# Balajimcr/MuLUT

Measured on AMD Instinct MI355X. Metric: Mpixels/sec SR-x4 2-stage sdy LUT inference (HR output pixels; LR-in = value/16), higher is better.
Workload: dtype u8; 1 GPU; 2-stage sdy x4, 128 x LR 1080x1920x3 -> HR 4320x7680x3 per GPU per step in 4 launches of 32 frames, D-natural; batch=32 draws, repeated in order to 128 frames, frames_per_gpu=128, frames_per_launch=32, stages=2, modes=sdy, scale=4, luts=shipped sr_x2sdy fine-tuned int8 tables, parallelism=frames sharded over 1 GPU(s), no collective

## Files before the change

mulut_amd/csrc/mulut_core.h:

```cpp
#ifndef MULUT_CORE_H_
#define MULUT_CORE_H_

#include <stdint.h>

#if defined(__HIPCC__)
#define MULUT_HD __host__ __device__ __forceinline__
#else
#define MULUT_HD static inline
#endif

namespace mulut {

template <int IV>
struct IvGeom {
    static_assert(IV >= 4 && IV <= 6, "sampling intervals 4, 5 and 6");
    static constexpr int q = 1 << IV;
    static constexpr int L = (1 << (8 - IV)) + 1;
    static constexpr int sA = L * L * L, sB = L * L, sC = L, sD = 1;
    static constexpr int rows = L * L * L * L;
    static constexpr int all = sA + sB + sC + sD;
};
MULUT_HD constexpr int interval_rows(int interval) {
    return interval == 4 ? IvGeom<4>::rows : interval == 5 ? IvGeom<5>::rows : interval == 6 ? IvGeom<6>::rows : 0;
}
// ... 532 lines not shown
    const uint32_t c0 = k0 & 0x0FFF0FFFu;
    const uint32_t c1 = c0 + (k1 & 0x0FFF0FFFu);
    const uint32_t c2 = c1 + (k2 & 0x0FFF0FFFu);
    o.cum[0] = pk_mad(pk_shr11(c0), pk_dup((uint32_t)kStrideA - kFullMark), c0);
    o.cum[1] = pk_mad(pk_shr11(c1), pk_dup((uint32_t)kStrideA - kFullMark), c1);
    o.cum[2] = pk_mad(pk_shr11(c2), pk_dup((uint32_t)kStrideA - kFullMark), c2);
    o.w[0] = pk_dup(kQ) - f1;
    o.w[1] = f1 - f2;
    o.w[2] = f2 - f3;
    o.w[3] = f3 - f4;
    o.w[4] = f4;
}
MULUT_HD void full_pair1_rows(const FullPair1 &p, int half, uint32_t (&r)[5]) {
    const uint32_t b = half ? (p.base >> 16) : (p.base & 0xFFFFu);
    r[0] = b;
    for (int j = 0; j < 3; ++j) {
        r[j + 1] = b + (half ? (p.cum[j] >> 16) : (p.cum[j] & 0xFFFFu));
    }
    r[4] = b + (uint32_t)kAllStrides;
}

MULUT_HD uint32_t bytes_3_1(uint32_t x) {
#if defined(__HIP_DEVICE_COMPILE__)
    return __builtin_amdgcn_perm(0u, x, 0x0C010C03u);
#else
    return (x >> 24) | (((x >> 8) & 0xFFu) << 16);
#endif
}
MULUT_HD uint32_t bytes_2_0(uint32_t x) {
#if defined(__HIP_DEVICE_COMPILE__)
    return __builtin_amdgcn_perm(0u, x, 0x0C000C02u);
#else
    return ((x >> 16) & 0xFFu) | ((x & 0xFFu) << 16);
#endif
}
MULUT_HD void swar_fma_rev4(uint32_t (&lo)[4], uint32_t (&hi)[4], const uint32_t (&row)[4], uint32_t w) {
    for (int k = 0; k < 4; ++k) {
        lo[3 - k] += bytes_3_1(row[k]) * w;
        hi[3 - k] += bytes_2_0(row[k]) * w;
    }
}

template <int HALF>
MULUT_HD void swar_fma_rev4_pk(uint32_t (&lo)[4], uint32_t (&hi)[4], const uint32_t (&row)[4], uint32_t wpk) {
    for (int k = 0; k < 4; ++k) {
        lo[3 - k] = pk_mad_w<HALF>(bytes_3_1(row[k]), wpk, lo[3 - k]);
        hi[3 - k] = pk_mad_w<HALF>(bytes_2_0(row[k]), wpk, hi[3 - k]);
    }
}

template <int HALF>
MULUT_HD uint32_t pk_mad_w_swap(uint32_t x, uint32_t wpk, uint32_t acc) {
#if defined(__HIP_DEVICE_COMPILE__)
    const mulut_u16x2 wv = MULUT_PK(wpk);
    const mulut_u16x2 ws = __builtin_shufflevector(wv, wv, HALF, HALF);
    const mulut_u16x2 xv = MULUT_PK(x);
    return MULUT_UNPK(__builtin_shufflevector(xv, xv, 1, 0) * ws + MULUT_PK(acc));
#else
    return pk_mad_w<HALF>((x >> 16) | (x << 16), wpk, acc);
#endif
}
template <int HALF>
MULUT_HD void swar_fma_x4(uint32_t (&lo)[4], uint32_t (&hi)[4], const uint32_t (&rlo)[4], const uint32_t (&rhi)[4], uint32_t wpk) {
    for (int k = 0; k < 4; ++k) {
        lo[k] = pk_mad_w<HALF>(rlo[k], wpk, lo[k]);
        hi[k] = pk_mad_w<HALF>(rhi[k], wpk, hi[k]);
    }
}
template <int HALF>
MULUT_HD void swar_fma_x4_rev(uint32_t (&lo)[4], uint32_t (&hi)[4], const uint32_t (&rlo)[4], const uint32_t (&rhi)[4], uint32_t wpk) {
    for (int k = 0; k < 4; ++k) {
        lo[3 - k] = pk_mad_w_swap<HALF>(rhi[k], wpk, lo[3 - k]);
        hi[3 - k] = pk_mad_w_swap<HALF>(rlo[k], wpk, hi[3 - k]);
    }
}

MULUT_HD void combine_pairs4(const uint32_t (&lo02)[4], const uint32_t (&hi02)[4], const uint32_t (&lo13)[4],
                             const uint32_t (&hi13)[4], uint32_t (&lo)[4], uint32_t (&hi)[4]) {
    lo[0] = lo02[0] + ((lo13[3] & 0xFFFFu) | (lo13[1] << 16));
    hi[0] = hi02[0] + ((lo13[2] & 0xFFFFu) | (lo13[0] << 16));
    lo[1] = lo02[1] + ((hi13[3] & 0xFFFFu) | (hi13[1] << 16));
    hi[1] = hi02[1] + ((hi13[2] & 0xFFFFu) | (hi13[0] << 16));
    lo[2] = lo02[2] + ((lo13[3] >> 16) | (lo13[1] & 0xFFFF0000u));
    hi[2] = hi02[2] + ((lo13[2] >> 16) | (lo13[0] & 0xFFFF0000u));
    lo[3] = lo02[3] + ((hi13[3] >> 16) | (hi13[1] & 0xFFFF0000u));
    hi[3] = hi02[3] + ((hi13[2] >> 16) | (hi13[0] & 0xFFFF0000u));
}

MULUT_HD uint32_t rhe_clip_u8_f32(int K, float inv_d) {
#if defined(__HIP_DEVICE_COMPILE__)
    const float q = __builtin_rintf((float)K * inv_d);
    return __builtin_amdgcn_cvt_pk_u8_f32(q, 0u, 0u);
#else
    const float q = __builtin_rintf((float)K * inv_d);
    return q < 0.0f ? 0u : (q > 255.0f ? 255u : (uint32_t)q);
#endif
}

MULUT_HD uint32_t rhe_pack4_f32(int K0, int K1, int K2, int K3, float inv_d) {
#if defined(__HIP_DEVICE_COMPILE__)
    uint32_t r = __builtin_amdgcn_cvt_pk_u8_f32(__builtin_rintf((float)K0 * inv_d), 0u, 0u);
    r = __builtin_amdgcn_cvt_pk_u8_f32(__builtin_rintf((float)K1 * inv_d), 1u, r);
    r = __builtin_amdgcn_cvt_pk_u8_f32(__builtin_rintf((float)K2 * inv_d), 2u, r);
    r = __builtin_amdgcn_cvt_pk_u8_f32(__builtin_rintf((float)K3 * inv_d), 3u, r);
    return r;
#else
    return rhe_clip_u8_f32(K0, inv_d) | (rhe_clip_u8_f32(K1, inv_d) << 8) | (rhe_clip_u8_f32(K2, inv_d) << 16) |
           (rhe_clip_u8_f32(K3, inv_d) << 24);
#endif
}

MULUT_HD uint32_t rhe_clip_u8_fma(uint32_t S, float inv_d, float c) {
    const float q = __builtin_rintf(__builtin_fmaf((float)S, inv_d, c));
#if defined(__HIP_DEVICE_COMPILE__)
    return __builtin_amdgcn_cvt_pk_u8_f32(q, 0u, 0u);
#else
    return q < 0.0f ? 0u : (q > 255.0f ? 255u : (uint32_t)q);
#endif
}
MULUT_HD uint32_t rhe_pack4_fma(uint32_t S0, uint32_t S1, uint32_t S2, uint32_t S3, float inv_d, float c) {
#if defined(__HIP_DEVICE_COMPILE__)
    uint32_t r = __builtin_amdgcn_cvt_pk_u8_f32(__builtin_fmaf((float)S0, inv_d, c), 0u, 0u);
    r = __builtin_amdgcn_cvt_pk_u8_f32(__builtin_fmaf((float)S1, inv_d, c), 1u, r);
    r = __builtin_amdgcn_cvt_pk_u8_f32(__builtin_fmaf((float)S2, inv_d, c), 2u, r);
    r = __builtin_amdgcn_cvt_pk_u8_f32(__builtin_fmaf((float)S3, inv_d, c), 3u, r);
    return r;
#else
    return rhe_clip_u8_fma(S0, inv_d, c) | (rhe_clip_u8_fma(S1, inv_d, c) << 8) | (rhe_clip_u8_fma(S2, inv_d, c) << 16) |
           (rhe_clip_u8_fma(S3, inv_d, c) << 24);
#endif
}
MULUT_HD bool rhe_fma_valid(uint32_t smax, int unbias, DivMagic m, float inv_d, float c) {
    for (uint32_t s = 0; s <= smax; ++s)
        if (rhe_clip_u8_fma(s, inv_d, c) != rhe_clip_u8((int)s - unbias, m)) return false;
    return true;
}

MULUT_HD uint32_t rhe_clip_u8_fma_i(int K, float inv_d, float c) {
    const float q = __builtin_rintf(__builtin_fmaf((float)K, inv_d, c));
    return q < 0.0f ? 0u : (q > 255.0f ? 255u : (uint32_t)q);
}
MULUT_HD bool rhe_fma_valid_i(int kmin, int kmax, int bias, DivMagic m, float inv_d, float c) {
    for (int k = kmin; k <= kmax; ++k)
        if (rhe_clip_u8_fma_i(k, inv_d, c) != rhe_clip_u8(k + bias, m)) return false;
    return true;
}

MULUT_HD bool rhe_f32_valid(int kmin, int kmax, DivMagic m, float inv_d) {
    for (int k = kmin; k <= kmax; ++k)
        if (rhe_clip_u8_f32(k, inv_d) != rhe_clip_u8(k, m)) return false;
    return true;
}

}
#endif
```

mulut_amd/csrc/mulut_kernels.hip:

```cpp
#include <hip/hip_runtime.h>
#include <string.h>

#include <mutex>
#include <set>
#include <utility>

#include "mulut_dev.h"
#include "mulut_interval.h"

namespace mulut {

template <int IV>
__device__ __forceinline__ int pass_value(const void *lut, int idx, int u, int e) {
    if (IV == kInterval && u > 1) return (int)((const uint8_t *)lut)[(long long)idx * (row_dwords(u) * 4) + e] - 128;
    return (int)((const int8_t *)lut)[(long long)idx * iv_row_bytes(u) + e];
}

template <int IV>
__global__ void __launch_bounds__(256) pass_kernel(PassArgs a) {
    const long long nsite = (long long)a.C * a.H * a.W;
    const long long s = (long long)blockIdx.x * blockDim.x + threadIdx.x;
    if (s >= nsite) return;
    const int x = (int)(s % a.W);
    const int y = (int)((s / a.W) % a.H);
// ... 394 lines not shown
    const uint32_t pd = w[(2 + yd) * PW + 2 + xd] | ((uint32_t)w[(2 - yd) * PW + 2 - xd] << 16);
    TubePair bp;
    simplex4_tube_pair<false>(k0, ha16, base_a, pb, pc, pd, bp);
    dirty |= bp.t_oob;
    tube_rows<R, 0, IMM>(smem, bp, acc);
    tube_rows<R + 2, 1, IMM>(smem, bp, acc);
}

template <int PAT, int PW>
__device__ __forceinline__ void tube_mode(const uint8_t *smem, uint32_t win, uint32_t k0, uint32_t ha16, uint32_t ha27, RotAcc<4> &acc, uint32_t &dirty) {
    const uint32_t base_a = ha27 + pk_dup((uint32_t)tube_bias(PAT));
    tube_pair<PAT, 0, PW>(smem, win, k0, ha16, base_a, acc, dirty);
    tube_pair<PAT, 1, PW>(smem, win, k0, ha16, base_a, acc, dirty);
}

template <int OUT, int TW, int TH>
__global__ void __launch_bounds__(TW *TH) stage_tube_kernel(StageArgs a, BandArgs b) {
    constexpr int PW = TW + 2 * kTubeHaloX, PH = TH + 2 * kHalo;
    constexpr int NT = TW * TH;
    constexpr int DW = PW / 4, PER4 = (3 * PH * DW + NT - 1) / NT;
    static_assert(((2 * 3 * PH * PW + 15) / 16) * 16 == kTubeTileBytes, "tile buffer size");
    extern __shared__ __attribute__((aligned(16))) uint8_t smem[];

    const int tx = threadIdx.x % TW, ty = threadIdx.x / TW;
    const int ntiles = a.N * a.tiles_x * a.tiles_y;
    const int G = gridDim.x;
    const bool by_xcd = (G & 7) == 0;
    const int per = (ntiles + 7) >> 3;
    const int first = by_xcd ? (int)(blockIdx.x & 7) * per + (int)(blockIdx.x >> 3) : (int)blockIdx.x;
    const int last = by_xcd ? imin(((int)(blockIdx.x & 7) + 1) * per, ntiles) : ntiles;
    const int step = by_xcd ? (G >> 3) : G;
    auto next_tile = [&](int t) {
        if (a.verdict_take >= 0)
            while (t < last && (int)a.verdict[t] != a.verdict_take) t += step;
        return t;
    };
    const int total = a.C * PH * PW;
    const int ylo = imax(a.oy0 - kHalo, 0), yhi = imin(a.oy1 + kHalo, a.H) - 1;
    const bool dw_ok = a.in.sX == 1 && ((a.W | a.in.sY | a.in.sC) & 3) == 0 && (a.in.sN & 3) == 0 && (((uintptr_t)a.in.p) & 3) == 0;
    auto fetch = [&](int tile, uint32_t (&v)[PER4]) {
        if (!dw_ok) return;
        int n, y0, x0;
        decode_tile(a, tile, n, y0, x0, TW, TH);
#pragma unroll
        for (int k = 0; k < PER4; ++k) {
            const int i = (int)threadIdx.x + k * NT;
            const int q = i % DW, py = (i / DW) % PH, c = imin(i / (DW * PH), a.C - 1);
            const int gy = imin(imax(y0 + py - kHalo, ylo), yhi);
            const int gx = imin(imax(x0 - kTubeHaloX + 4 * q, 0), a.W - 4);
            v[k] = *(const uint32_t *)view_addr(a.in, n, c, gy, gx);
        }
    };
    auto stash = [&](int tile, int buf, const uint32_t (&v)[PER4]) {
        int n, y0, x0;
        decode_tile(a, tile, n, y0, x0, TW, TH);
        uint8_t *dst = smem + 3 * kTubeBandBytes + buf * kTubeTileBytes;
        if (dw_ok) {
            int tid = (int)threadIdx.x;
            asm volatile("" : "+v"(tid));
#pragma unroll
            for (int k = 0; k < PER4; ++k) {
                const int i = tid + k * NT;
                if (i < a.C * PH * DW) {
                    const int gx = x0 - kTubeHaloX + 4 * (i % DW);
                    const uint32_t sel_lo = gx < 0 ? 0x0C000C00u : gx > a.W - 4 ? 0x0C030C03u : 0x0C010C00u;
                    const uint32_t sel_hi = gx < 0 ? 0x0C000C00u : gx > a.W - 4 ? 0x0C030C03u : 0x0C030C02u;
                    const uint32_t lo = __builtin_amdgcn_perm(0u, v[k], sel_lo), hi = __builtin_amdgcn_perm(0u, v[k], sel_hi);
                    uint2 c2;
                    c2.x = pk_mad(lo, pk_dup(0x1001u), 0u) & 0xF0F0F0F0u;
                    c2.y = pk_mad(hi, pk_dup(0x1001u), 0u) & 0xF0F0F0F0u;
                    *(uint2 *)(dst + 8 * i) = c2;
                }
            }
        } else {
            for (int i = threadIdx.x; i < total; i += NT) {
                const int px = i % PW, py = (i / PW) % PH, c = i / (PW * PH);
                const int gy = imin(imax(y0 + py - kHalo, ylo), yhi);
                const int gx = imin(imax(x0 + px - kTubeHaloX, 0), a.W - 1);
                ((uint16_t *)dst)[i] = (uint16_t)pixel_code(*view_addr(a.in, n, c, gy, gx));
            }
        }
    };

    int tile = next_tile(first);
    if (tile >= last) return;
    uint32_t pix[PER4];
    fetch(tile, pix);
    for (int m = 0; m < a.M; ++m) {
        const int pat = a.dj[m][0] == 2 ? 1 : a.di[m][0] == 1 ? 2 : 0;
        const uint4 *src = (const uint4 *)b.band[m];
        uint4 *dst = (uint4 *)(smem + pat * kTubeBandBytes);
        for (int i = threadIdx.x; i < kTubeBandBytes / 16; i += NT) dst[i] = src[i];
    }
    stash(tile, 0, pix);
    __syncthreads();

    for (int it = 0; tile < last; ++it) {
        const int nxt = next_tile(tile + step);
        if (nxt < last) fetch(nxt, pix);
        int n, y0, x0;
        decode_tile(a, tile, n, y0, x0, TW, TH);
        const int y = y0 + ty, x = x0 + tx;
        if (y < a.oy1 && x < a.W) {
            uint32_t win = (uint32_t)(3 * kTubeBandBytes + (it & 1) * kTubeTileBytes + 2 * (ty * PW + tx + kTubeHaloX - kHalo));
            uint32_t o0[4], o1[4], o2[4];
#pragma unroll
            for (int k = 0; k < 4; ++k) o0[k] = o1[k] = o2[k] = 0;
            uint32_t dmask = 0u;
#pragma clang loop unroll(disable)
            for (int c = 0; c < a.C; ++c, win += 2 * PH * PW) {
                uint32_t dirty = 0u;
                const uint32_t ca = *(const uint16_t *)(smem + win + 2 * (2 * PW + 2));
                const uint32_t k0 = tube_anchor_key(ca), ha16 = tube_anchor_h16(ca), ha27 = pk_mad(ha16, pk_dup(kTubeSA), 0u);
                RotAcc<4> acc;
                acc.clear();
                for (int mv = 0; mv < a.M; ++mv) {
                    const int m = __builtin_amdgcn_readfirstlane(mv);
                    const int pat = a.dj[m][0] == 2 ? 1 : a.di[m][0] == 1 ? 2 : 0;
                    if (pat == 0) tube_mode<0, PW>(smem, win, k0, ha16, ha27, acc, dirty);
                    else if (pat == 1) tube_mode<1, PW>(smem, win, k0, ha16, ha27, acc, dirty);
                    else tube_mode<2, PW>(smem, win, k0, ha16, ha27, acc, dirty);
                }
                if constexpr (OUT == kOutPackedRGBU4) {
#pragma unroll
                    for (int k = 0; k < 4; ++k) { o0[k] = o1[k]; o1[k] = o2[k]; }
                    tube_finish_rows(a, acc, o2);
                } else {
                    uint32_t o[4];
                    finish_channel<4, OUT>(a, acc, n, c, y, x, o);
                }
                dmask |= (dirty != 0u ? 1u : 0u) << c;
            }
            if constexpr (OUT == kOutPackedRGBU4) store_rgb<4>(a, n, y, x, o0, o1, o2);
            if (__ballot(dmask != 0u) != 0ull) {
                const uint32_t pixel_id = ((uint32_t)n * (uint32_t)a.H + (uint32_t)y) * (uint32_t)a.W + (uint32_t)x;
                for (int c = 0; c < a.C; ++c) {
                    const bool d = ((dmask >> c) & 1u) != 0u;
                    const unsigned long long dm = __ballot(d);
                    if (dm == 0ull) continue;
                    const int lane = (int)(threadIdx.x & 63);
                    uint32_t at = 0;
                    if (lane == __ffsll((long long)dm) - 1) at = atomicAdd(a.fix_count, (uint32_t)__popcll(dm));
                    at = (uint32_t)__shfl((int)at, __ffsll((long long)dm) - 1);
                    if (d) a.fix_list[at + (uint32_t)__popcll(dm & ((1ull << lane) - 1ull))] = pixel_id | ((uint32_t)c << 30);
                }
            }
        }
        if (nxt < last) stash(nxt, (it + 1) & 1, pix);
        __syncthreads();
        tile = nxt;
    }
}

__global__ void __launch_bounds__(256) stage_up_fix2_kernel(StageArgs a) {
    __shared__ int s_sum[16][16];
    const uint32_t count = *a.fix_count;
    const int grp = (int)(threadIdx.x >> 4), ln = (int)(threadIdx.x & 15);
    const int ylo = imax(a.oy0 - kHalo, 0), yhi = imin(a.oy1 + kHalo, a.H) - 1;
    const int unbias = 128 * kQ * 4 * a.M - a.bias_num;
    for (uint32_t i = blockIdx.x * 16u + (uint32_t)grp; i < count; i += gridDim.x * 16u) {
        const uint32_t ent = a.fix_list[i], id = ent & 0x3FFFFFFFu, only = ent >> 30;
        const int x = (int)(id % (uint32_t)a.W), y = (int)((id / (uint32_t)a.W) % (uint32_t)a.H), n = (int)(id / ((uint32_t)a.W * (uint32_t)a.H));
        if (n >= a.N || y < a.oy0 || y >= a.oy1) continue;
        const int c_lo = only == 3u ? 0 : (int)only, c_hi = only == 3u ? imin(a.C, 3) : imin((int)only + 1, a.C);
        for (int c = c_lo; c < c_hi; ++c) {
            s_sum[grp][ln] = 0;
            __builtin_amdgcn_fence(__ATOMIC_RELEASE, "wavefront");
            auto px = [&](int dy, int dx) {
                const int gy = imin(imax(y + dy, ylo), yhi), gx = imin(imax(x + dx, 0), a.W - 1);
                return (int)*view_addr(a.in, n, c, gy, gx);
            };
            const int va = px(0, 0);
            for (int p = ln; p < 4 * a.M; p += 16) {
                const int m = p >> 2, r = p & 3;
                int dy, dx, v[3];
#pragma unroll
                for (int k = 0; k < 3; ++k) {
                    sample_offset(r, a.di[m][k], a.dj[m][k], dy, dx);
                    v[k] = px(dy, dx);
                }
                int idx[5], w[5];
                simplex4(va, v[0], v[1], v[2], idx, w);
                const uint4 *tab = (const uint4 *)a.lut[m];
                uint32_t row[5][4];
#pragma unroll
                for (int j = 0; j < 5; ++j) {
                    const uint4 t = tab[idx[j]];
                    row[j][0] = t.x; row[j][1] = t.y; row[j][2] = t.z; row[j][3] = t.w;
                }
#pragma unroll
                for (int e = 0; e < 16; ++e) {
                    int sum = 0;
#pragma unroll
                    for (int j = 0; j < 5; ++j) sum += w[j] * (int)((row[j][e >> 2] >> (8 * (e & 3))) & 0xFFu);
                    const int pos = r == 0 ? e : r == 1 ? (e & 3) * 4 + 3 - (e >> 2) : r == 2 ? 15 - e : (3 - (e & 3)) * 4 + (e >> 2);
                    atomicAdd(&s_sum[grp][pos], sum);
                }
            }
            __builtin_amdgcn_fence(__ATOMIC_ACQ_REL, "wavefront");
            const uint32_t b = rhe_clip_u8(s_sum[grp][ln] - unbias, a.div);
            *const_cast<uint8_t *>(view_addr(a.out, n, c, y * 4 + (ln >> 2), x * 4 + (ln & 3))) = (uint8_t)b;
            __builtin_amdgcn_fence(__ATOMIC_ACQ_REL, "wavefront");
        }
    }
}

hipError_t launch_stage_up_fix(const StageArgs &a, int num_cus, hipStream_t st) {
    if (a.C > 3 || !a.fix_list || !a.fix_count) return hipErrorInvalidValue;
    hipLaunchKernelGGL(stage_up_fix2_kernel, dim3((unsigned)(8 * num_cus)), dim3(256), 0, st, a);
    return hipGetLastError();
}

const char *stage_tube_name(int out_mode) {
    return out_mode == kOutPackedRGBU4 ? "stage_tube_kernel<rgb>" : out_mode == kOutPlanarU4 ? "stage_tube_kernel<planar>"
                                                                                              : "stage_tube_kernel<generic>";
}

template <int OUT>
static hipError_t launch_tube_t(const StageArgs &a, const BandArgs &b, int num_cus, hipStream_t st) {
    auto kern = stage_tube_kernel<OUT, KB_TW, KB_TH>;
    {
        const hipError_t e = raise_lds_limit((const void *)kern, 160 * 1024);
        if (e != hipSuccess) return e;
    }
    const long long ntiles = (long long)a.N * a.tiles_x * a.tiles_y;
    if (ntiles <= 0 || ntiles > 0x7fffffffLL) return hipErrorInvalidValue;
    const unsigned grid = (unsigned)(ntiles < num_cus ? ntiles : num_cus);
    hipLaunchKernelGGL(kern, dim3(grid), dim3(KB_TW * KB_TH), (size_t)kTubeLdsBytes, st, a, b);
    return hipGetLastError();
}

hipError_t launch_stage_tube(const StageArgs &a, const BandArgs &b, int out_mode, int num_cus, hipStream_t st) {
    if (a.C > 3 || a.M > 3) return hipErrorInvalidValue;
    if (out_mode == kOutPlanarU4) return launch_tube_t<kOutPlanarU4>(a, b, num_cus, st);
    if (out_mode == kOutPackedRGBU4 && a.C == 3) return launch_tube_t<kOutPackedRGBU4>(a, b, num_cus, st);
    return launch_tube_t<kOutGeneric>(a, b, num_cus, st);
}

#if defined(MULUT_TUBE2_ASM_INC)
#include MULUT_TUBE2_ASM_INC
#else
#include "mulut_tube2_asm.inc"
#endif

struct T2Pair {
    uint32_t base, s0, s1, s2;
    uint32_t w0, w1, w2, w3, w4;
};
__host__ __device__ constexpr int t2_modes(int pats) { return pats & 3; }
__host__ __device__ constexpr int t2_pat(int pats, int m) { return (pats >> (2 + 2 * m)) & 3; }
constexpr int kT2W = 16, kT2H = 4;
constexpr int kT2PW = kT2W + 2 * kTubeHaloX, kT2PH = kT2H + 2 * kHalo, kT2Chan = 2 * kT2PH * kT2PW;
constexpr int kT2WaveTileBytes = 3 * kT2Chan;
constexpr int kT2FixCap = 3 * kT2W * kT2H;
constexpr int kT2FixOff = 3 * kTubeBandBytes + 16 * kT2WaveTileBytes + 2 * 16 * KB_TW * KB_TH;
constexpr int kTube2LdsBytes = kT2FixOff + 16 * kT2FixCap * 4 + 16;
static_assert(kTube2LdsBytes <= 160 * 1024, "LDS budget");
static_assert(KB_TW % kT2W == 0 && KB_TH % kT2H == 0 && (KB_TW / kT2W) * (KB_TH / kT2H) == 16 && KB_TW / kT2W == 4, "16 wave tiles per verdict tile, four across");
__host__ __device__ constexpr int t2_nb(int pat, int r, int k, int sign) {
    return 2 * ((2 + sign * rot_dy(r, kPatDi[pat][k], kPatDj[pat][k])) * kT2PW + 2 + sign * rot_dx(r, kPatDi[pat][k], kPatDj[pat][k]));
}
__host__ __device__ constexpr int t2_imm(int pat) { return pat * kTubeBandBytes - tube_bias(pat); }

__device__ __forceinline__ float t2_f32_of_i16(uint32_t x) {
    float f;
    asm("v_cvt_f32_i32_sdwa %0, sext(%1) dst_sel:DWORD dst_unused:UNUSED_PAD src0_sel:WORD_0" : "=v"(f) : "v"(x));
    return f;
}

template <int PAT>
__device__ __forceinline__ void t2_index(uint32_t k0, uint32_t ha, uint32_t base_a0, uint32_t pb, uint32_t pc, uint32_t pd, T2Pair &o, uint32_t &dirty, bool test) {
    constexpr uint32_t SB = kTubeSB * 16, SC = kTubeSC * 16, SD = kTubeSD * 16;
    uint32_t k1 = pb | pk_dup(SB), k2 = pc | pk_dup(SC), k3 = pd | pk_dup(SD);
    pk_cmpx_desc(k0, k1);
    pk_cmpx_desc(k2, k3);
    pk_cmpx_desc(k0, k2);
    pk_cmpx_desc(k1, k3);
    pk_cmpx_desc(k1, k2);
    const uint32_t f1 = pk_shr12(k0), f2 = pk_shr12(k1), f3 = pk_shr12(k2), f4 = pk_shr12(k3);
    o.base = pk_mad(pb, pk_dup(SB), pk_mad(pc, pk_dup(SC), pk_mad(pd, pk_dup(SD), base_a0 + pk_dup((uint32_t)tube_bias(PAT)))));
    o.s0 = k0 & 0x0FF00FF0u;
    o.s1 = k1 & 0x0FF00FF0u;
    o.s2 = k2 & 0x0FF00FF0u;
    o.w0 = pk_dup(kQ) - f1;
    o.w1 = f1 - f2;
    o.w2 = f2 - f3;
    o.w3 = f3 - f4;
    o.w4 = f4;
    if (test) {
        asm volatile("; MULUT_T2_TUBE_TEST");
        const uint32_t hb = pb & 0x000F000Fu, hc = pc & 0x000F000Fu, hd = pd & 0x000F000Fu;
        const uint32_t mx = pk_max(pk_max(hb, hc), pk_max(hd, ha));
        const uint32_t mn = pk_min(pk_min(hb, hc), pk_min(hd, ha));
        dirty |= (mx - mn) & 0xFFFEFFFEu;
    }
}

#define T2_ACC_OPS(lo, hi) [l0] "+v"(lo[0]), [l1] "+v"(lo[1]), [l2] "+v"(lo[2]), [l3] "+v"(lo[3]), [h0] "+v"(hi[0]), [h1] "+v"(hi[1]), [h2] "+v"(hi[2]), [h3] "+v"(hi[3])
#define T2_TMP_OPS [a0] "=&v"(a0), [a1] "=&v"(a1), [a2] "=&v"(a2), [a3] "=&v"(a3)
#define T2_W_OPS(c) [w0] "v"(c.w0), [w1] "v"(c.w1), [w2] "v"(c.w2), [w3] "v"(c.w3), [w4] "v"(c.w4)
#define T2_ADDR_OPS(n) [base] "v"(n.base), [s0] "v"(n.s0), [s1] "v"(n.s1), [s2] "v"(n.s2)
#define T2_IMM_OPS(PAT) [ilo] "i"(t2_imm(PAT)), [ihi] "i"(t2_imm(PAT) + kTubePlaneBytes), [ilo4] "i"(t2_imm(PAT) + kTubeAll * 16), [ihi4] "i"(t2_imm(PAT) + kTubeAll * 16 + kTubePlaneBytes)
#define T2_NB_OPS(PAT, R, OFF) [n0] "i"(t2_nb(PAT, R, 0, 1) + (OFF)), [n1] "i"(t2_nb(PAT, R, 0, -1) + (OFF)), [n2] "i"(t2_nb(PAT, R, 1, 1) + (OFF)), \
    [n3] "i"(t2_nb(PAT, R, 1, -1) + (OFF)), [n4] "i"(t2_nb(PAT, R, 2, 1) + (OFF)), [n5] "i"(t2_nb(PAT, R, 2, -1) + (OFF)), [nan] "i"(2 * (2 * kT2PW + 2) + (OFF))

#define T2_NBOUT_OPS [pb] "=&v"(pb), [pc] "=&v"(pc), [pd] "=&v"(pd), [t0] "=&v"(t0), [t1] "=&v"(t1), [t2] "=&v"(t2)
template <int PAT, int FORM>
__device__ __forceinline__ void t2_block_a(uint32_t (&lo)[4], uint32_t (&hi)[4], const T2Pair &cur) {
    uint32_t a0, a1, a2, a3;
#define T2_A_STMT(BLK) asm volatile(BLK : T2_ACC_OPS(lo, hi), T2_TMP_OPS : T2_W_OPS(cur), T2_ADDR_OPS(cur), T2_IMM_OPS(PAT) : TUBE2_CLOBBERS)
    if constexpr (FORM < 0) T2_A_STMT(TUBE2_ASM_A);
    else if constexpr (FORM == 0) T2_A_STMT(TUBE2_ASM1_A_R0);
    else T2_A_STMT(TUBE2_ASM1_A_R1);
#undef T2_A_STMT
}
template <int FORM, int NPAT, int NN, int TPAT, int TR, int TOFF, bool LAST>
__device__ __forceinline__ void t2_block_b(uint32_t (&lo)[4], uint32_t (&hi)[4], const T2Pair &cur, const T2Pair &nxt, uint32_t win,
                                           uint32_t &pb, uint32_t &pc, uint32_t &pd, uint32_t &ca) {
    uint32_t a0, a1, a2, a3, t0, t1, t2;
#define T2_B_STMTS(BLK)                                                                                                                                       \
    do {                                                                                                                                                      \
        if constexpr (LAST)                                                                                                                                   \
            asm volatile(BLK##_LAST : T2_ACC_OPS(lo, hi) : T2_W_OPS(cur) : TUBE2_CLOBBERS);                                                                  \
        else if constexpr (NN == 0)                                                                                                                           \
            asm volatile(BLK##_N0 : T2_ACC_OPS(lo, hi), T2_TMP_OPS : T2_W_OPS(cur), T2_ADDR_OPS(nxt), T2_IMM_OPS(NPAT) : TUBE2_CLOBBERS);                    \
        else if constexpr (NN == 6)                                                                                                                           \
            asm volatile(BLK##_N6 : T2_ACC_OPS(lo, hi), T2_TMP_OPS, T2_NBOUT_OPS : T2_W_OPS(cur), T2_ADDR_OPS(nxt), T2_IMM_OPS(NPAT), [win] "v"(win), T2_NB_OPS(TPAT, TR, TOFF) : TUBE2_CLOBBERS); \
        else                                                                                                                                                  \
            asm volatile(BLK##_N7 : T2_ACC_OPS(lo, hi), T2_TMP_OPS, T2_NBOUT_OPS, [ca] "=&v"(ca) : T2_W_OPS(cur), T2_ADDR_OPS(nxt), T2_IMM_OPS(NPAT), [win] "v"(win), T2_NB_OPS(TPAT, TR, TOFF) : TUBE2_CLOBBERS); \
    } while (0)
    if constexpr (FORM < 0) T2_B_STMTS(TUBE2_ASM_B);
    else if constexpr (FORM == 0) T2_B_STMTS(TUBE2_ASM1_B_R0);
    else T2_B_STMTS(TUBE2_ASM1_B_R1);
#undef T2_B_STMTS
}

template <int FORM, int NPAT, int NN, int TPAT, int TR, int TOFF, bool LAST>
__device__ __forceinline__ void t2_block_b_either(uint32_t (&lo)[4], uint32_t (&hi)[4], const T2Pair &cur, const T2Pair &nxt, uint32_t win, uint32_t more,
                                                  uint32_t &pb, uint32_t &pc, uint32_t &pd, uint32_t &ca) {
    static_assert((FORM == 0 || FORM == 1) && (NN == 6 || NN == 7), "one-set blocks");
    uint32_t a0, a1, a2, a3, t0, t1, t2;
#define T2_E6_STMT(BLK)                                                                                  \
    asm volatile(BLK : T2_ACC_OPS(lo, hi), T2_TMP_OPS, T2_NBOUT_OPS                                      \
                 : T2_W_OPS(cur), T2_ADDR_OPS(nxt), T2_IMM_OPS(NPAT), [win] "v"(win), T2_NB_OPS(TPAT, TR, TOFF), [more] "s"(more) : TUBE2_CLOBBERS, "scc")
#define T2_E7_STMT(BLK)                                                                                  \
    asm volatile(BLK : T2_ACC_OPS(lo, hi), T2_TMP_OPS, T2_NBOUT_OPS, [ca] "=&v"(ca)                      \
                 : T2_W_OPS(cur), T2_ADDR_OPS(nxt), T2_IMM_OPS(NPAT), [win] "v"(win), T2_NB_OPS(TPAT, TR, TOFF), [more] "s"(more) : TUBE2_CLOBBERS, "scc")
    if constexpr (FORM == 0 && NN == 6 && !LAST) T2_E6_STMT(TUBE2_ASM1_B_R0_N6_OR_N0);
    else if constexpr (FORM == 0 && NN == 6) T2_E6_STMT(TUBE2_ASM1_B_R0_N6_OR_LAST);
    else if constexpr (FORM == 0 && !LAST) T2_E7_STMT(TUBE2_ASM1_B_R0_N7_OR_N0);
    else if constexpr (FORM == 0) T2_E7_STMT(TUBE2_ASM1_B_R0_N7_OR_LAST);
    else if constexpr (NN == 6 && !LAST) T2_E6_STMT(TUBE2_ASM1_B_R1_N6_OR_N0);
    else if constexpr (NN == 6) T2_E6_STMT(TUBE2_ASM1_B_R1_N6_OR_LAST);
    else if constexpr (!LAST) T2_E7_STMT(TUBE2_ASM1_B_R1_N7_OR_N0);
    else T2_E7_STMT(TUBE2_ASM1_B_R1_N7_OR_LAST);
#undef T2_E6_STMT
#undef T2_E7_STMT
// ... 424 lines not shown
```

Measured before the change: 151,600 Mpix/s.

## Add specialized fix2 path with packed byte MAC and fewer LDS atomics

Adds a fast path for the stage upsampling fix-up kernel when there are at most four modes and the input offsets fit in 32 bits. It replaces the 16 per-element LDS atomic adds with packed-byte multiply-accumulate and eight rotated dword LDS atomics per lane. It also swaps the 64-bit index division for magic-reciprocal decoding, precomputes the sample offsets per lane, and pins occupancy with waves_per_eu. The fix-up list is probably small, so the kernel may be only a minor share of total runtime.

```diff
diff --git a/mulut_amd/csrc/mulut_core.h b/mulut_amd/csrc/mulut_core.h
--- a/mulut_amd/csrc/mulut_core.h
+++ b/mulut_amd/csrc/mulut_core.h
@@ -708,5 +708,65 @@
     return true;
 }
 
-}
-#endif
+MULUT_HD uint32_t fix2_odd_bytes(uint32_t d) {
+#if defined(__HIP_DEVICE_COMPILE__)
+    return __builtin_amdgcn_perm(0u, d, 0x0C030C01u);
+#else
+    return (d >> 8) & 0x00FF00FFu;
+#endif
+}
+MULUT_HD void fix2_mac_row(uint32_t (&F)[4], uint32_t (&H)[4], const uint32_t (&row)[4], uint32_t w) {
+    for (int k = 0; k < 4; ++k) {
+        F[k] = pk_mad_w<0>(row[k], w, F[k]);
+        H[k] = pk_mad_w<0>(fix2_odd_bytes(row[k]), w, H[k]);
+    }
+}
+MULUT_HD void fix2_pass_sums(const uint32_t (&F)[4], const uint32_t (&H)[4], uint32_t (&X)[8]) {
+    for (int k = 0; k < 4; ++k) {
+        X[k] = slab_even_sums(F[k], H[k]);
+        X[4 + k] = H[k];
+    }
+}
+MULUT_HD constexpr int fix2_slot(int r, int j) { return (r & 1) * 8 + (j ^ ((r & 2) ? 7 : 0)); }
+MULUT_HD constexpr uint32_t fix2_swap(int r) { return (r & 2) ? 16u : 0u; }
+MULUT_HD uint32_t fix2_rotr(uint32_t x, uint32_t s) {
+#if defined(__HIP_DEVICE_COMPILE__)
+    return __builtin_amdgcn_alignbit(x, x, s);
+#else
+    return s ? (x >> 16) | (x << 16) : x;
+#endif
+}
+MULUT_HD constexpr int fix2_partner(int p) { return 12 + (p >> 2) - 4 * (p & 3); }
+MULUT_HD constexpr int fix2_field_half(int set, int E) { return set * 16 + ((E & 1) * 4 + (E >> 2)) * 2 + ((E >> 1) & 1); }
+
+struct Recip30 {
+    uint32_t d, magic, shift, exact;
+};
+MULUT_HD Recip30 make_recip30(uint32_t d) {
+    Recip30 r;
+    r.d = d;
+    r.magic = r.shift = r.exact = 0;
+    if (d < 2) return r;
+    r.shift = (uint32_t)(30 - __builtin_clz(d));
+    const uint64_t p = 1ull << (32 + r.shift), m = (p + d - 1) / d, e = m * d - p;
+    r.magic = (uint32_t)m;
+    r.exact = ((m >> 32) == 0 && e * ((1ull << 30) - 1) < p) ? 1u : 0u;
+    return r;
+}
+MULUT_HD uint32_t recip30_div(uint32_t id, const Recip30 &r) { return (uint32_t)(((uint64_t)id * r.magic) >> 32) >> r.shift; }
+MULUT_HD void fix2_decode(uint32_t id, uint32_t W, uint32_t H, const Recip30 &rw, const Recip30 &rwh, bool fast, int &x, int &y, int &n) {
+    uint32_t row, img;
+    if (fast) {
+        row = recip30_div(id, rw);
+        img = recip30_div(id, rwh);
+    } else {
+        row = id / W;
+        img = id / (W * H);
+    }
+    x = (int)(id - row * W);
+    y = (int)(row - img * H);
+    n = (int)img;
+}
+
+}
+#endif
diff --git a/mulut_amd/csrc/mulut_kernels.hip b/mulut_amd/csrc/mulut_kernels.hip
--- a/mulut_amd/csrc/mulut_kernels.hip
+++ b/mulut_amd/csrc/mulut_kernels.hip
@@ -570,8 +570,20 @@
     }
 }
 
-__global__ void __launch_bounds__(256) stage_up_fix2_kernel(StageArgs a) {
-    __shared__ int s_sum[16][16];
+template <int K>
+__device__ __forceinline__ uint32_t add_byte_k(uint32_t a, uint32_t b) {
+    static_assert(K >= 0 && K < 3, "byte 0, 1 or 2");
+    uint32_t r;
+    if constexpr (K == 0) asm("v_add_u32_sdwa %0, %1, %2 dst_sel:DWORD dst_unused:UNUSED_PAD src0_sel:DWORD src1_sel:BYTE_0" : "=v"(r) : "v"(a), "v"(b));
+    if constexpr (K == 1) asm("v_add_u32_sdwa %0, %1, %2 dst_sel:DWORD dst_unused:UNUSED_PAD src0_sel:DWORD src1_sel:BYTE_1" : "=v"(r) : "v"(a), "v"(b));
+    if constexpr (K == 2) asm("v_add_u32_sdwa %0, %1, %2 dst_sel:DWORD dst_unused:UNUSED_PAD src0_sel:DWORD src1_sel:BYTE_2" : "=v"(r) : "v"(a), "v"(b));
+    return r;
+}
+__device__ __forceinline__ void lds_add_u32(uint32_t addr, uint32_t v) {
+    __hip_atomic_fetch_add((__attribute__((address_space(3))) uint32_t *)(uintptr_t)addr, v, __ATOMIC_RELAXED, __HIP_MEMORY_SCOPE_WORKGROUP);
+}
+
+__device__ __forceinline__ void fix2_any_modes(const StageArgs &a, int (&s_sum)[16][16]) {
     const uint32_t count = *a.fix_count;
     const int grp = (int)(threadIdx.x >> 4), ln = (int)(threadIdx.x & 15);
     const int ylo = imax(a.oy0 - kHalo, 0), yhi = imin(a.oy1 + kHalo, a.H) - 1;
@@ -621,6 +633,87 @@
             __builtin_amdgcn_fence(__ATOMIC_ACQ_REL, "wavefront");
         }
     }
+}
+
+
+__device__ __forceinline__ void fix2_four_modes(const StageArgs &a, int (&s_sum)[16][16]) {
+    const uint32_t count = *a.fix_count;
+    const int grp = (int)(threadIdx.x >> 4), ln = (int)(threadIdx.x & 15);
+    const int ylo = imax(a.oy0 - kHalo, 0), yhi = imin(a.oy1 + kHalo, a.H) - 1;
+    const int unbias = 128 * kQ * 4 * a.M - a.bias_num;
+    const bool act = ln < 4 * a.M;
+    const int m = act ? ln >> 2 : 0, r = ln & 3;
+    uint32_t dy4 = 0u, dx4 = 0u;
+#pragma unroll
+    for (int k = 0; k < 3; ++k) {
+        int dy, dx;
+        sample_offset(r, a.di[m][k], a.dj[m][k], dy, dx);
+        dy4 |= (uint32_t)(dy + 4) << (8 * k);
+        dx4 |= (uint32_t)(dx + 4) << (8 * k);
+    }
+    const char *tab = (const char *)a.lut[m];
+    uint32_t *sum = (uint32_t *)s_sum[grp];
+    const uint32_t dst0 = lds_addr_of(sum + fix2_slot(r, 0));
+    const uint32_t swap = fix2_swap(r);
+    const uint16_t *f02 = (const uint16_t *)sum + fix2_field_half(0, ln), *f13 = (const uint16_t *)sum + fix2_field_half(1, fix2_partner(ln));
+    const uint32_t W = (uint32_t)a.W, H = (uint32_t)a.H;
+    const Recip30 rw = make_recip30(W), rwh = make_recip30(W * H);
+    const bool fast = rw.exact != 0 && rwh.exact != 0;
+    const uint32_t sY = (uint32_t)a.in.sY, sX = (uint32_t)a.in.sX;
+    for (uint32_t i = blockIdx.x * 16u + (uint32_t)grp; i < count; i += gridDim.x * 16u) {
+        const uint32_t ent = a.fix_list[i], id = ent & 0x3FFFFFFFu, only = ent >> 30;
+        int x, y, n;
+        fix2_decode(id, W, H, rw, rwh, fast, x, y, n);
+        if (n >= a.N || y < a.oy0 || y >= a.oy1) continue;
+        const int c_lo = (int)only - 3 * (int)((only + 1u) >> 2), c_hi = imin(imin(a.C, 3), (int)only + 1);
+        const uint8_t *src = a.in.p + (long long)n * a.in.sN + (long long)c_lo * a.in.sC;
+        const uint8_t *pa = src + ((uint32_t)(y - a.in.row0) * sY + (uint32_t)x * sX), *pk[3];
+        const uint32_t y4 = (uint32_t)(y - 4), x4 = (uint32_t)(x - 4);
+        static_for<0, 3>([&](auto K) {
+            const int gy = imin(imax((int)add_byte_k<K>(y4, dy4), ylo), yhi), gx = imin(imax((int)add_byte_k<K>(x4, dx4), 0), a.W - 1);
+            pk[K] = src + ((uint32_t)(gy - a.in.row0) * sY + (uint32_t)gx * sX);
+        });
+        uint8_t *out = const_cast<uint8_t *>(view_addr(a.out, n, c_lo, y * 4 + (ln >> 2), x * 4 + (ln & 3)));
+        for (int c = c_lo; c < c_hi; ++c, pa += a.in.sC, pk[0] += a.in.sC, pk[1] += a.in.sC, pk[2] += a.in.sC, out += a.out.sC) {
+            sum[ln] = 0;
+            __builtin_amdgcn_fence(__ATOMIC_RELEASE, "wavefront");
+            const int va = (int)*pa;
+            if (act) {
+                const int v0 = (int)*pk[0], v1 = (int)*pk[1], v2 = (int)*pk[2];
+                int idx[5], w[5];
+                simplex4(va, v0, v1, v2, idx, w);
+                uint32_t row[5][4];
+#pragma unroll
+                for (int j = 0; j < 5; ++j) {
+                    const uint4 t = *(const uint4 *)(tab + ((uint32_t)idx[j] << 4));
+                    row[j][0] = t.x; row[j][1] = t.y; row[j][2] = t.z; row[j][3] = t.w;
+                }
+                uint32_t F[4] = {0u, 0u, 0u, 0u}, Hs[4] = {0u, 0u, 0u, 0u}, X[8];
+#pragma unroll
+                for (int j = 0; j < 5; ++j) fix2_mac_row(F, Hs, row[j], (uint32_t)w[j]);
+                fix2_pass_sums(F, Hs, X);
+                uint32_t d0 = dst0;
+                asm volatile("" : "+v"(d0));
+                static_for<0, 8>([&](auto J) { lds_add_u32(d0 ^ (uint32_t)(4 * J), fix2_rotr(X[J], swap)); });
+            }
+            __builtin_amdgcn_fence(__ATOMIC_ACQ_REL, "wavefront");
+            const uint32_t b = rhe_clip_u8((int)((uint32_t)*f02 + (uint32_t)*f13) - unbias, a.div);
+            *out = (uint8_t)b;
+            __builtin_amdgcn_fence(__ATOMIC_ACQ_REL, "wavefront");
+        }
+    }
+}
+
+__device__ __forceinline__ bool fix2_offsets_fit(const StageArgs &a) {
+    const int ylo = imax(a.oy0 - kHalo, 0), yhi = imin(a.oy1 + kHalo, a.H) - 1;
+    if (a.in.sY < 0 || a.in.sX < 0 || ylo < a.in.row0 || yhi < ylo || a.W < 1) return false;
+    return (unsigned long long)(yhi - a.in.row0) * (unsigned long long)a.in.sY + (unsigned long long)(a.W - 1) * (unsigned long long)a.in.sX < (1ull << 32);
+}
+
+__global__ void __launch_bounds__(256) __attribute__((amdgpu_waves_per_eu(8, 8))) stage_up_fix2_kernel(StageArgs a) {
+    __shared__ __attribute__((aligned(64))) int s_sum[16][16];
+    if (a.M <= 4 && fix2_offsets_fit(a)) fix2_four_modes(a, s_sum);
+    else fix2_any_modes(a, s_sum);
 }
 
 hipError_t launch_stage_up_fix(const StageArgs &a, int num_cus, hipStream_t st) {
```

After: 153,500 Mpix/s (median of 6 runs). +1.3%, better.
